# aai-institute/USFlows

Hardware: AMD Instinct MI355X
Metric: log_prob samples/sec (whole node), 32-layer 784-dim flow, batch 65536 (higher is better)
Workload: dtype f32 (GEMMs as bf16x3 split on the bf16 MFMA: 24 significant bits, fp32 accumulate); 1 GPU; BASELINE cfg2: USFlow in_dims=[784], 32 additive coupling blocks, ConditionalDenseNN[256, 256]+LeakyReLU(0.01), lu_transform=1, householder=0, affine_conjugation=False, Laplace(0,1) base; log_prob of 65536 rows per GPU (65536 over 1 GPU(s)) resident in HBM; conditioned synthetic parameters (seed 100, alpha 0.1); rows_per_gpu=65536, global_rows=65536, parallelism=dp1 (single GPU: no collective), fused_coupling=True, gemm_mode=bf16x3, merge_affine=auto -> False; probe (accepted, element-wise, L1) []

## Files before the change

### usflows_amd/csrc/usf_coupling_planes.hip

```cpp
#include <stdlib.h>

#include <type_traits>

#include "usf_common.h"

namespace usf {

typedef __bf16 cp_bf16x8 __attribute__((ext_vector_type(8)));
typedef _Float16 cp_f16x8 __attribute__((ext_vector_type(8)));
#define USF_CP_F16_GUARD 65000.0f
#ifndef USF_CP_ADDR32
#define USF_CP_ADDR32 1
#endif

__device__ __forceinline__ void cp_pin(unsigned& off) { asm("" : "+v"(off)); }
template <class V> __device__ __forceinline__ V cp_load(const void* uniform, unsigned off) {
  return *reinterpret_cast<const V*>(reinterpret_cast<const char*>(uniform) + off);
}
template <class V> __device__ __forceinline__ void cp_store(void* uniform, unsigned off, const V v) {
  *reinterpret_cast<V*>(reinterpret_cast<char*>(uniform) + off) = v;
}

__device__ __forceinline__ float max_with_product(float x, float sx) {
  float r;
  asm("v_max_f32 %0, %1, %2" : "=v"(r) : "v"(x), "v"(sx));
  return r;
}

template <int NPL> struct CPlanes;
template <> struct CPlanes<3> {
  typedef cp_bf16x8 vec;
  static __device__ __forceinline__ f32x4 mfma(vec a, vec b, f32x4 c) { return __builtin_amdgcn_mfma_f32_16x16x32_bf16(a, b, c, 0, 0, 0); }
  static __device__ __forceinline__ void split(const f32x4 x0, const f32x4 x1, vec (&o)[3]) {
#pragma unroll
    for (int j = 0; j < 8; ++j) {
      const float x = (j < 4) ? x0[j & 3] : x1[j & 3];
      const __bf16 h = (__bf16)x;
      const float r = x - (float)h;
      const __bf16 m = (__bf16)r;
      o[0][j] = h; o[1][j] = m; o[2][j] = (__bf16)(r - (float)m);
    }
  }
  static __device__ __forceinline__ void split1(const float x, const int j, vec (&o)[3]) {
    const __bf16 h = (__bf16)x;
    const float r = x - (float)h;
    const __bf16 m = (__bf16)r;
    o[0][j] = h; o[1][j] = m; o[2][j] = (__bf16)(r - (float)m);
  }
  static __device__ __forceinline__ void mm(f32x4& acc, const vec (&w)[3], const vec (&a)[3]) {
    acc = mfma(w[2], a[0], acc); acc = mfma(w[1], a[1], acc); acc = mfma(w[0], a[2], acc);
    acc = mfma(w[1], a[0], acc); acc = mfma(w[0], a[1], acc); acc = mfma(w[0], a[0], acc);
  }
};
template <> struct CPlanes<2> {
  typedef cp_f16x8 vec;
  static __device__ __forceinline__ f32x4 mfma(vec a, vec b, f32x4 c) { return __builtin_amdgcn_mfma_f32_16x16x32_f16(a, b, c, 0, 0, 0); }
  static __device__ __forceinline__ void split(const f32x4 x0, const f32x4 x1, vec (&o)[2]) {
#pragma unroll
    for (int j = 0; j < 8; ++j) {
      const float x = (j < 4) ? x0[j & 3] : x1[j & 3];
      const _Float16 h = (_Float16)x;
      o[0][j] = h; o[1][j] = (_Float16)(x - (float)h);
    }
  }
  static __device__ __forceinline__ void split1(const float x, const int j, vec (&o)[2]) {
    const _Float16 h = (_Float16)x;
    o[0][j] = h; o[1][j] = (_Float16)(x - (float)h);
  }
  static __device__ __forceinline__ void mm(f32x4& acc, const vec (&w)[2], const vec (&a)[2]) {
    acc = mfma(w[1], a[0], acc); acc = mfma(w[0], a[1], acc); acc = mfma(w[0], a[0], acc);
  }
};

struct CplPArgs {
  char* z; int z_nkb, npanels, M;
  int kb_p0, nk_p, kb_t0, nk_t;
  const char* Win; int64_t ld_in, pl_in; const float* b_in;
  const char* Whid[2]; int64_t ld_hid, pl_hid; const float* b_hid[2];
  const char* Wout; int64_t ld_out, pl_out; const float* b_out;
  float sign, slope; int act;
  int act_max;
  int32_t* range_flag;
  int descend;
  unsigned long long* dbg;
  char* hout[2]; const char* gate[2];
  const float* ctx; int ctx_stride; const float* w_ctx; const float* b_ctx;
  const char* side;
};

#ifdef USF_STAMP
#define CSTAMP(v) unsigned long long v = __builtin_amdgcn_s_memtime(); __builtin_amdgcn_sched_barrier(0)
#else
#define CSTAMP(v)
#endif

template <int NPL, int NH, int MODE = 0, bool CTX = false, bool SIDE = false>
__global__ __launch_bounds__(512, 2) void coupling_planes_kernel(const CplPArgs p) {
  static_assert(!SIDE || (MODE == 0 && !CTX), "the fp32 residual serves the plain inference launch");
  typedef CPlanes<NPL> PT;
  typedef typename PT::vec vec8;
  constexpr int T = 16;
  constexpr int HP = 16 * T;
  constexpr int KS = T / 2;
  constexpr int NT = 512;
  constexpr int SLOTS = NPL * 4 * HP;
  constexpr int NST = SLOTS / NT;
  constexpr int NPP = NST / NPL;
  constexpr int NC = HP / 8;
  constexpr int NPR = (NPL == 3) ? 6 : 3;
#ifndef USF_CP_AHEAD
#define USF_CP_AHEAD 3
#endif
  constexpr int AHEAD = USF_CP_AHEAD;
  __shared__ __attribute__((aligned(16))) float lds[2][SLOTS * 4];

  const int tid = threadIdx.x;
  const int lane = tid & 63;
  constexpr bool A32 = USF_CP_ADDR32 != 0;
  const int wave = A32 ? __builtin_amdgcn_readfirstlane(tid >> 6) : (tid >> 6);
  const int lj = lane & 15, lg = lane >> 4;
  unsigned loff = (unsigned)lane * 16u;
  unsigned goff = (unsigned)lg * 16u;
  const int panel = (p.descend ? (int)(gridDim.x - 1 - blockIdx.x) : (int)blockIdx.x) * 8 + wave;
  const int panc = min(panel, p.npanels - 1);
  const bool live = panel < p.npanels;
  const bool live_z = CTX ? (live && 16 * panel + lj < p.M) : live;
  const f32x4 zero4 = {0.f, 0.f, 0.f, 0.f};
  constexpr unsigned CHB = NPL * 1024u;
  const size_t zbase = ((size_t)panc * p.z_nkb) * CHB + (size_t)lane * 16;
  char* const zrow = p.z + ((size_t)panc * p.z_nkb) * CHB;
  auto k_off = [&](int64_t ld) { return 2u * ((unsigned)(tid >> 2) * (unsigned)ld + 8u * (unsigned)(tid & 3)); };
  auto n_off = [&](int64_t ld) { return 2u * ((unsigned)(tid / NC) * (unsigned)ld + 8u * (unsigned)(tid % NC)); };

  int kdst[NPP];
  unsigned krow[NPP];
#pragma unroll
  for (int i = 0; i < NPP; ++i) {
    const int idx = tid + NT * i;
    const int r = idx >> 2, c = idx & 3;
    kdst[i] = 4 * (c * HP + (r ^ (2 * c)));
    krow[i] = (unsigned)r;
  }
  auto issue_k = [&](const char* W, int64_t ld, int64_t pl, int k0, unsigned& off, f32x4 (&st)[NST]) {
    if constexpr (A32) cp_pin(off);
#pragma unroll
    for (int q = 0; q < NPL; ++q)
#pragma unroll
      for (int i = 0; i < NPP; ++i) {
        if constexpr (A32)
          st[q * NPP + i] = cp_load<f32x4>(W + 2 * (q * pl + (int64_t)((NT / 4) * i) * ld + k0), off);
        else
          st[q * NPP + i] = *reinterpret_cast<const f32x4*>(W + 2 * (q * pl + (int64_t)krow[i] * ld + k0 + 8 * ((tid + NT * i) & 3)));
      }
  };
  auto store_k = [&](int buf, const f32x4 (&st)[NST]) {
#pragma unroll
    for (int q = 0; q < NPL; ++q)
#pragma unroll
      for (int i = 0; i < NPP; ++i) *reinterpret_cast<f32x4*>(&lds[buf][q * 16 * HP + kdst[i]]) = st[q * NPP + i];
  };
  auto n_rc = [&](int i, int& r, int& c) { const int idx = tid + NT * i; r = idx / NC; c = idx % NC; };
  auto issue_n = [&](const char* W, int64_t ld, int64_t pl, int n0, unsigned& off, f32x4 (&st)[NST]) {
    if constexpr (A32) cp_pin(off);
#pragma unroll
    for (int q = 0; q < NPL; ++q)
#pragma unroll
      for (int i = 0; i < NPP; ++i) {
        if constexpr (A32) {
          st[q * NPP + i] = cp_load<f32x4>(W + 2 * (q * pl + (int64_t)(n0 + (NT / NC) * i) * ld), off);
        } else {
          int r, c; n_rc(i, r, c);
          st[q * NPP + i] = *reinterpret_cast<const f32x4*>(W + 2 * (q * pl + (int64_t)(n0 + r) * ld + 8 * c));
        }
      }
  };
  auto store_n = [&](int buf, const f32x4 (&st)[NST]) {
#pragma unroll
    for (int q = 0; q < NPL; ++q)
#pragma unroll
      for (int i = 0; i < NPP; ++i) {
        int r, c; n_rc(i, r, c);
        *reinterpret_cast<f32x4*>(&lds[buf][4 * ((q * NC + c) * 32 + (r ^ (2 * (c & 7))))]) = st[q * NPP + i];
      }
  };

  auto bias4 = [&](const float* b, int t) {
    if constexpr (A32) { if (t == 0) cp_pin(goff); return cp_load<f32x4>(b + t * 16, goff); }
    else return *reinterpret_cast<const f32x4*>(b + t * 16 + 4 * lg);
  };
  f32x4 X1[T], X2[T];
#pragma unroll
  for (int t = 0; t < T; ++t) X1[t] = bias4(p.b_in, t);
  if (CTX) {
    const int crow = min(16 * panc + lj, p.M - 1);
    const float c = p.ctx[(size_t)crow * p.ctx_stride];
#pragma unroll
    for (int t = 0; t < T; ++t) {
      const f32x4 wc = *reinterpret_cast<const f32x4*>(p.w_ctx + t * 16 + 4 * lg);
      const f32x4 bc = *reinterpret_cast<const f32x4*>(p.b_ctx + t * 16 + 4 * lg);
#pragma unroll
      for (int e = 0; e < 4; ++e) X1[t][e] = __builtin_fmaf(c, wc[e], X1[t][e] + bc[e]);
    }
  }

  auto load_z = [&](int kb, vec8 (&dst)[NPL]) {
    if constexpr (A32) cp_pin(loff);
#pragma unroll
    for (int q = 0; q < NPL; ++q) {
      if constexpr (A32) dst[q] = cp_load<vec8>(zrow + ((size_t)(p.kb_p0 + kb) * CHB + q * 1024), loff);
      else dst[q] = *reinterpret_cast<const vec8*>(p.z + zbase + (size_t)(p.kb_p0 + kb) * CHB + q * 1024);
    }
  };

  auto mfma_slab = [&](int buf, f32x4 (&X)[T], const vec8 (&b)[NPL]) {
    const float* wl = &lds[buf][4 * (lg * HP + (lj ^ (2 * lg)))];
#pragma unroll
    for (int ht = 0; ht < T; ++ht) {
      vec8 w[NPL];
#pragma unroll
      for (int q = 0; q < NPL; ++q) w[q] = *reinterpret_cast<const vec8*>(wl + 4 * ((q * 4) * HP + ht * 16));
#ifndef USF_CP_NOPRIO
      if (ht & 1) __builtin_amdgcn_s_setprio(0); else __builtin_amdgcn_s_setprio(1);
#endif
      PT::mm(X[ht], w, b);
    }
  };
#define CP_PIN_SLAB(NLD, VPT)                                                                     \
  do {                                                                                            \
    __builtin_amdgcn_sched_group_barrier(0x100, NPL * AHEAD, 0);                                  \
    _Pragma("unroll") for (int ht_ = 0; ht_ < T; ++ht_) {                                         \
      __builtin_amdgcn_sched_group_barrier(0x008, NPR, 0);                                        \
      if (ht_ + AHEAD < T) __builtin_amdgcn_sched_group_barrier(0x100, NPL, 0);                   \
      if (ht_ < (NLD)) __builtin_amdgcn_sched_group_barrier(0x020, 1, 0);                         \
      if (ht_ >= 3 && (VPT) > 0) __builtin_amdgcn_sched_group_barrier(0x002, (VPT), 0);           \
    }                                                                                             \
  } while (0)

  bool bad = false;
  auto guard = [&](const f32x4 v) {
    if (NPL == 2) {
#pragma unroll
      for (int j = 0; j < 4; ++j) bad = bad || !(fabsf(v[j]) < USF_CP_F16_GUARD);
    }
  };

  CSTAMP(c0);
  int g = 0;
  f32x4 st[NST];
  vec8 zp[NPL], zn[NPL];
  unsigned koff_in = k_off(p.ld_in), koff_hid = k_off(p.ld_hid), noff = n_off(p.ld_out);
  issue_k(p.Win, p.ld_in, p.pl_in, 0, koff_in, st);
  load_z(0, zp);
  store_k(0, st);
  __syncthreads();

  for (int s = 0; s + 1 < p.nk_p; ++s, ++g) {
    const int buf = g & 1;
    issue_k(p.Win, p.ld_in, p.pl_in, (s + 1) * 32, koff_in, st);
    load_z(s + 1, zn);
    mfma_slab(buf, X1, zp);
    CP_PIN_SLAB(NST + NPL, 0);
    __builtin_amdgcn_sched_barrier(0);
    store_k(buf ^ 1, st);
#pragma unroll
    for (int q = 0; q < NPL; ++q) zp[q] = zn[q];
    __syncthreads();
  }
  {
    const int buf = g & 1;
    if (NH >= 2) issue_k(p.Whid[0], p.ld_hid, p.pl_hid, 0, koff_hid, st); else issue_n(p.Wout, p.ld_out, p.pl_out, 0, noff, st);
    mfma_slab(buf, X1, zp);
    CP_PIN_SLAB(NST, 0);
    __builtin_amdgcn_sched_barrier(0);
    if (NH >= 2) store_k(buf ^ 1, st); else store_n(buf ^ 1, st);
    __syncthreads();
    ++g;
  }
  const size_t hbase = (size_t)panc * 8 * CHB + (size_t)lane * 16;
  const size_t hrow = (size_t)panc * 8 * CHB;
  auto activate = [&](f32x4 (&X)[T], int l) {
    if (MODE == 2) {
      if constexpr (A32) cp_pin(loff);
#pragma unroll
      for (int ks = 0; ks < KS; ++ks) {
        const vec8 hv = A32 ? cp_load<vec8>(p.gate[l] + (hrow + (size_t)ks * CHB), loff)
                            : *reinterpret_cast<const vec8*>(p.gate[l] + hbase + (size_t)ks * CHB);
#pragma unroll
        for (int t = 0; t < 4; ++t) {
          X[2 * ks][t] = gate_apply(X[2 * ks][t], (float)hv[t], p.slope);
          X[2 * ks + 1][t] = gate_apply(X[2 * ks + 1][t], (float)hv[4 + t], p.slope);
        }
      }
      return;
    }
    if (p.act_max) {
#pragma unroll
      for (int ht = 0; ht < T; ++ht) {
#pragma unroll
        for (int t = 0; t < 4; ++t) X[ht][t] = max_with_product(X[ht][t], X[ht][t] * p.slope);
        guard(X[ht]);
      }
      return;
    }
#pragma unroll
    for (int ht = 0; ht < T; ++ht) {
#pragma unroll
      for (int t = 0; t < 4; ++t) X[ht][t] = act_apply(X[ht][t], p.act, p.slope);
      guard(X[ht]);
    }
  };
  auto save_hidden = [&](int l, int ks, const vec8 (&x)[NPL]) {
    if (MODE != 0 && live) {
      if constexpr (A32) cp_pin(loff);
#pragma unroll
      for (int q = 0; q < NPL; ++q) {
        if constexpr (A32) cp_store<vec8>(p.hout[l] + (hrow + (size_t)ks * CHB + q * 1024), loff, x[q]);
        else *reinterpret_cast<vec8*>(p.hout[l] + hbase + (size_t)ks * CHB + q * 1024) = x[q];
      }
    }
  };
  activate(X1, 0);
  CSTAMP(c1);

  auto hidden_layer = [&](f32x4 (&Xin)[T], f32x4 (&Xout)[T], int l) {
    vec8 xc[NPL], xn[NPL];
    PT::split(Xin[0], Xin[1], xc);
#pragma unroll
    for (int ks = 0; ks < KS; ++ks) {
      save_hidden(l, ks, xc);
      const int buf = g & 1;
      const bool last = (ks + 1 == KS);
      const bool next_is_hidden = (l + 2 < NH);
      if (!last) issue_k(p.Whid[l], p.ld_hid, p.pl_hid, (ks + 1) * 32, koff_hid, st);
      else if (next_is_hidden) issue_k(p.Whid[l + 1], p.ld_hid, p.pl_hid, 0, koff_hid, st);
      else issue_n(p.Wout, p.ld_out, p.pl_out, 0, noff, st);
      mfma_slab(buf, Xout, xc);
      if (!last) PT::split(Xin[2 * ks + 2], Xin[2 * ks + 3], xn);
      CP_PIN_SLAB(NST, (NPL == 3) ? 5 : 3);
      __builtin_amdgcn_sched_barrier(0);
      if (!last || next_is_hidden) store_k(buf ^ 1, st); else store_n(buf ^ 1, st);
      if (!last) {
#pragma unroll
        for (int q = 0; q < NPL; ++q) xc[q] = xn[q];
      }
      __syncthreads();
      ++g;
    }
    activate(Xout, l + 1);
  };
  if (NH >= 2) {
#pragma unroll
    for (int t = 0; t < T; ++t) X2[t] = bias4(p.b_hid[0], t);
    hidden_layer(X1, X2, 0);
  }
  if (NH >= 3) {
#pragma unroll
    for (int t = 0; t < T; ++t) X1[t] = bias4(p.b_hid[1], t);
    hidden_layer(X2, X1, 1);
  }

  CSTAMP(c2);
  auto output_layer = [&](f32x4 (&X)[T]) {
    vec8 xp[KS][NPL];
#pragma unroll
    for (int ks = 0; ks < KS; ++ks) { PT::split(X[2 * ks], X[2 * ks + 1], xp[ks]); save_hidden(NH - 1, ks, xp[ks]); }
    typename std::conditional<SIDE, f32x4, vec8>::type res[SIDE ? 2 : NPL];
    f32x4 bo[2];
    unsigned soff = (unsigned)lane * 32u;
    const char* const srow = SIDE ? p.side + ((size_t)panc * p.nk_t) * 2048u : nullptr;
    auto issue_res = [&](int nt) {
      if constexpr (A32) { cp_pin(loff); cp_pin(goff); }
      if constexpr (SIDE) {
        if constexpr (A32) cp_pin(soff);
#pragma unroll
        for (int u = 0; u < 2; ++u) res[u] = cp_load<f32x4>(srow + ((size_t)nt * 2048u + 16 * u), soff);
      } else {
#pragma unroll
        for (int q = 0; q < NPL; ++q) {
          if constexpr (A32) res[q] = cp_load<vec8>(zrow + ((size_t)(p.kb_t0 + nt) * CHB + q * 1024), loff);
          else res[q] = *reinterpret_cast<const vec8*>(p.z + zbase + (size_t)(p.kb_t0 + nt) * CHB + q * 1024);
        }
      }
#pragma unroll
      for (int u = 0; u < 2; ++u) {
        if constexpr (A32) bo[u] = cp_load<f32x4>(p.b_out + nt * 32 + 16 * u, goff);
        else bo[u] = *reinterpret_cast<const f32x4*>(p.b_out + nt * 32 + 16 * u + 4 * lg);
      }
    };
    auto epilogue = [&](int nt, const auto& ac, const auto& rs) {
      f32x4 v[2];
#pragma unroll
      for (int u = 0; u < 2; ++u) {
#pragma unroll
        for (int e = 0; e < 4; ++e) {
          float r;
          if constexpr (SIDE) {
            r = rs[u][e];
          } else {
            r = (float)rs[0][4 * u + e] + (float)rs[1][4 * u + e];
            if (NPL == 3) r = r + (float)rs[NPL - 1][4 * u + e];
          }
          v[u][e] = __builtin_fmaf(p.sign, ac[u][e], r);
        }
        guard(v[u]);
      }
      vec8 o[NPL];
      PT::split(v[0], v[1], o);
      if (live_z) {
        if constexpr (A32) cp_pin(loff);
#pragma unroll
        for (int q = 0; q < NPL; ++q) {
          if constexpr (A32) cp_store<vec8>(zrow + ((size_t)(p.kb_t0 + nt) * CHB + q * 1024), loff, o[q]);
          else *reinterpret_cast<vec8*>(p.z + zbase + (size_t)(p.kb_t0 + nt) * CHB + q * 1024) = o[q];
        }
      }
    };
    issue_res(0);
    auto block = [&](int nt) {
      const int buf = g & 1;
      issue_n(p.Wout, p.ld_out, p.pl_out, min(nt + 1, p.nk_t - 1) * 32, noff, st);
      f32x4 acc[2] = {bo[0], bo[1]};
#pragma unroll
      for (int ks = 0; ks < KS; ++ks) {
        const int x = 2 * ((4 * ks + lg) & 7);
#pragma unroll
        for (int u = 0; u < 2; ++u) {
          const float* wf = &lds[buf][4 * ((4 * ks + lg) * 32 + u * 16 + (lj ^ x))];
          vec8 w[NPL];
#pragma unroll
          for (int q = 0; q < NPL; ++q) w[q] = *reinterpret_cast<const vec8*>(wf + 4 * (q * NC * 32));
          PT::mm(acc[u], w, xp[ks]);
        }
      }
      __builtin_amdgcn_sched_group_barrier(0x100, NPL * AHEAD, 0);
#pragma unroll
      for (int i = 0; i < 2 * KS; ++i) {
        __builtin_amdgcn_sched_group_barrier(0x008, NPR, 0);
        if (i + AHEAD < 2 * KS) __builtin_amdgcn_sched_group_barrier(0x100, NPL, 0);
        if (i < NST + (SIDE ? 2 : NPL) + 2) __builtin_amdgcn_sched_group_barrier(0x020, 1, 0);
      }
      __builtin_amdgcn_sched_barrier(0);
      store_n(buf ^ 1, st);
      epilogue(nt, acc, res);
      issue_res(min(nt + 1, p.nk_t - 1));
      __syncthreads();
      ++g;
    };
    for (int nt = 0; nt < p.nk_t; ++nt) block(nt);
  };
  if (NH == 2) output_layer(X2); else output_layer(X1);
#ifdef USF_STAMP
  CSTAMP(c3);
  if (p.dbg && lane == 0) {
    unsigned long long* o = p.dbg + (size_t)((blockIdx.x % 2048) * 8 + wave) * 4;
    o[0] = c1 - c0; o[1] = c2 - c1; o[2] = c3 - c2; o[3] = 1;
  }
#endif
  if (NPL == 2 && p.range_flag && bad && live && (16 * panel + lj) < p.M) atomicOr(p.range_flag, 1);
#undef CP_PIN_SLAB
}



#ifdef USF_STAMP
unsigned long long* g_cdbg = nullptr;
#endif

static int coupling_planes_launch(const usf_coupling_planes_desc* d, const float* ctx, int64_t ctx_stride, const float* w_ctx,
                                  const float* b_ctx, const void* side, int64_t side_nkb, hipStream_t stream) {
  if (!d) { set_error("usf_coupling_planes: null descriptor"); return -1; }
  if (ctx) {
    if (d->act == USF_ACT_GATE) { set_error("usf_coupling_planes_ctx: USF_ACT_GATE takes no context (the context enters no data gradient)"); return -2; }
    if (ctx_stride != 0 && ctx_stride != 1) { set_error("usf_coupling_planes_ctx: ctx_stride must be 0 or 1 (got %lld)", (long long)ctx_stride); return -2; }
    if (!w_ctx || !b_ctx || !aligned16(w_ctx) || !aligned16(b_ctx)) {
      set_error("usf_coupling_planes_ctx: w_ctx / b_ctx must be [256] fp32 vectors, 16-byte aligned");
      return -2;
    }
  }
  if (d->M < 0 || d->M > 0x7fffffff || d->z_nkb <= 0 || d->n_hidden < 1 || d->n_hidden > 3 || d->nk_p <= 0 || d->nk_t <= 0 ||
      d->kb_p0 < 0 || d->kb_t0 < 0 || d->kb_p0 + d->nk_p > d->z_nkb || d->kb_t0 + d->nk_t > d->z_nkb) {
    set_error("usf_coupling_planes: bad sizes / block ranges");
    return -2;
  }
  if (d->M == 0) return 0;
  if (d->format != USF_PLANES_BF16X3 && d->format != USF_PLANES_F16X2) { set_error("usf_coupling_planes: unknown format %d", d->format); return -2; }
  if (!d->z || !d->W_in || !d->W_out || !d->b_in || !d->b_out) { set_error("usf_coupling_planes: null pointer"); return -1; }
  for (int i = 0; i + 1 < d->n_hidden; ++i)
    if (!d->W_hid[i] || !d->b_hid[i]) { set_error("usf_coupling_planes: hidden layer %d missing", i); return -1; }
  if (d->hidden_padded != 256) { set_error("usf_coupling_planes: weights must be padded to a hidden width of 256 (got %d)", d->hidden_padded); return -2; }
  if (d->ldw_in < 32 * d->nk_p || (d->n_hidden > 1 && d->ldw_hid < 256) || d->ldw_out < 256 || (d->ldw_in & 7) || (d->ldw_hid & 7) ||
      (d->ldw_out & 7) || !aligned16(d->z) || !aligned16(d->W_in) || !aligned16(d->W_out) || !aligned16(d->b_in) || !aligned16(d->b_out)) {
    set_error("usf_coupling_planes: weight-image contract violated (ldw_in >= 32 nk_p, ldw_hid / ldw_out >= 256, multiples of 8, 16-byte aligned)");
    return -2;
  }
  const int64_t npl = d->format == USF_PLANES_F16X2 ? 2 : 3;
  const int64_t npanels = (d->M + 15) / 16;
  if (2 * npl * d->w_in_plane >= (1LL << 40)) { set_error("usf_coupling_planes: operand too large"); return -3; }
  {
    const int64_t lim = 1LL << 32, chb = npl * 1024;
    const bool z_big = d->z_nkb >= lim / chb || npanels * d->z_nkb * chb >= lim;
    const bool h_big = (d->hidden_out[0] || d->hidden_out[1]) && npanels * 8 * chb >= lim;
    auto w_big = [&](int64_t ld, int64_t plane, int64_t rows) {
      return ld < 0 || plane < 0 || ld >= lim / (2 * rows) || plane >= lim / (2 * npl);
    };
    if (z_big || h_big || w_big(d->ldw_in, d->w_in_plane, 256) || (d->n_hidden > 1 && w_big(d->ldw_hid, d->w_hid_plane, 256)) ||
        w_big(d->ldw_out, d->w_out_plane, 32 * d->nk_t)) {
      set_error("usf_coupling_planes: a buffer of 4 GiB or more (z: %lld panels x %lld blocks x %lld bytes; weights: ld %lld / %lld / %lld)",
                (long long)npanels, (long long)d->z_nkb, (long long)chb, (long long)d->ldw_in, (long long)d->ldw_hid, (long long)d->ldw_out);
      return -3;
    }
  }
  if (side) {
    if (ctx || d->hidden_out[0] || d->hidden_out[1] || d->act == USF_ACT_GATE) {
      set_error("usf_coupling_planes_side: the fp32 residual serves the inference launch without a context (no hidden_out, no USF_ACT_GATE)");
      return -2;
    }
    if (!aligned16(side)) { set_error("usf_coupling_planes_side: side must be 16-byte aligned"); return -2; }
    if (side_nkb != d->nk_t) {
      set_error("usf_coupling_planes_side: the side buffer holds %lld blocks per panel, the layer transforms %lld", (long long)side_nkb, (long long)d->nk_t);
      return -2;
    }
    if (npanels * d->nk_t * 2048 >= (1LL << 32)) { set_error("usf_coupling_planes_side: side buffer of 4 GiB or more"); return -3; }
  }
  CplPArgs a;
  a.side = reinterpret_cast<const char*>(side);
  a.z = reinterpret_cast<char*>(d->z); a.z_nkb = (int)d->z_nkb; a.npanels = (int)npanels; a.M = (int)d->M;
  a.kb_p0 = (int)d->kb_p0; a.nk_p = (int)d->nk_p; a.kb_t0 = (int)d->kb_t0; a.nk_t = (int)d->nk_t;
  a.Win = reinterpret_cast<const char*>(d->W_in); a.ld_in = d->ldw_in; a.pl_in = d->w_in_plane; a.b_in = d->b_in;
  for (int i = 0; i < 2; ++i) {
    const bool used = i + 1 < d->n_hidden;
    a.Whid[i] = reinterpret_cast<const char*>(used ? d->W_hid[i] : d->W_in);
    a.b_hid[i] = used ? d->b_hid[i] : d->b_in;
  }
  a.ld_hid = d->ldw_hid; a.pl_hid = d->w_hid_plane;
  a.Wout = reinterpret_cast<const char*>(d->W_out); a.ld_out = d->ldw_out; a.pl_out = d->w_out_plane; a.b_out = d->b_out;
  a.sign = d->sign; a.slope = d->slope; a.act = d->act; a.range_flag = d->range_flag;
  a.act_max = (d->act == USF_ACT_LEAKY_RELU && d->slope >= 0.0f && d->slope <= 1.0f && !__builtin_signbit(d->slope) &&
               tuning("coupling_act_max", 1) != 0) ? 1 : 0;
  a.descend = (int)tuning("coupling_descend", 1);
  a.ctx = ctx; a.ctx_stride = (int)ctx_stride; a.w_ctx = w_ctx; a.b_ctx = b_ctx;
  a.dbg = nullptr;
#ifdef USF_STAMP
  a.dbg = g_cdbg;
#endif
  const dim3 grid((unsigned)((npanels + 7) / 8));
  const bool want_h = d->hidden_out[0] != nullptr || d->hidden_out[1] != nullptr;
  const bool gated = d->act == USF_ACT_GATE;
  if (d->act != USF_ACT_NONE && d->act != USF_ACT_LEAKY_RELU && !gated) { set_error("usf_coupling_planes: bad act %d", d->act); return -2; }
  for (int i = 0; i < 2; ++i) { a.hout[i] = nullptr; a.gate[i] = nullptr; }
  if (want_h || gated) {
    if (npl != 3 || d->n_hidden > 2) { set_error("usf_coupling_planes: hidden_out / USF_ACT_GATE need the bf16x3 format and n_hidden <= 2"); return -2; }
    if (gated && !want_h) { set_error("usf_coupling_planes: USF_ACT_GATE needs hidden_out (the gradients at the hidden pre-activations)"); return -2; }
    for (int i = 0; i < d->n_hidden; ++i) {
      if (!d->hidden_out[i] || !aligned16(d->hidden_out[i]) || (gated && (!d->gate[i] || !aligned16(d->gate[i])))) {
        set_error("usf_coupling_planes: hidden_out[l] (and gate[l] with USF_ACT_GATE) must be set for every hidden layer, 16-byte aligned");
        return -2;
      }
      a.hout[i] = reinterpret_cast<char*>(d->hidden_out[i]);
      a.gate[i] = reinterpret_cast<const char*>(gated ? d->gate[i] : nullptr);
    }
    const dim3 block(512);
#define USF_CPT(NH_, MODE_) hipLaunchKernelGGL((coupling_planes_kernel<3, NH_, MODE_>), grid, block, 0, stream, a)
#define USF_CPTC(NH_) hipLaunchKernelGGL((coupling_planes_kernel<3, NH_, 1, true>), grid, block, 0, stream, a)
    if (gated) { if (d->n_hidden == 1) USF_CPT(1, 2); else USF_CPT(2, 2); }
    else if (ctx) { if (d->n_hidden == 1) USF_CPTC(1); else USF_CPTC(2); }
    else { if (d->n_hidden == 1) USF_CPT(1, 1); else USF_CPT(2, 1); }
#undef USF_CPTC
#undef USF_CPT
    return check_launch("usf_coupling_planes");
  }
  const dim3 block(512);
#define USF_CPL(NPL_, NH_) hipLaunchKernelGGL((coupling_planes_kernel<NPL_, NH_>), grid, block, 0, stream, a)
#define USF_CPLC(NPL_, NH_) hipLaunchKernelGGL((coupling_planes_kernel<NPL_, NH_, 0, true>), grid, block, 0, stream, a)
#define USF_CPLS(NPL_, NH_) hipLaunchKernelGGL((coupling_planes_kernel<NPL_, NH_, 0, false, true>), grid, block, 0, stream, a)
  if (side) {
    if (npl == 2) {
      switch (d->n_hidden) { case 1: USF_CPLS(2, 1); break; case 2: USF_CPLS(2, 2); break; default: USF_CPLS(2, 3); break; }
    } else {
      switch (d->n_hidden) { case 1: USF_CPLS(3, 1); break; case 2: USF_CPLS(3, 2); break; default: USF_CPLS(3, 3); break; }
    }
  } else if (ctx) {
    if (npl == 2) {
      switch (d->n_hidden) { case 1: USF_CPLC(2, 1); break; case 2: USF_CPLC(2, 2); break; default: USF_CPLC(2, 3); break; }
    } else {
      switch (d->n_hidden) { case 1: USF_CPLC(3, 1); break; case 2: USF_CPLC(3, 2); break; default: USF_CPLC(3, 3); break; }
    }
  } else if (npl == 2) {
    switch (d->n_hidden) { case 1: USF_CPL(2, 1); break; case 2: USF_CPL(2, 2); break; default: USF_CPL(2, 3); break; }
  } else {
    switch (d->n_hidden) { case 1: USF_CPL(3, 1); break; case 2: USF_CPL(3, 2); break; default: USF_CPL(3, 3); break; }
  }
#undef USF_CPLS
#undef USF_CPLC
#undef USF_CPL
  return check_launch("usf_coupling_planes");
}

int coupling_planes_ctx(const usf_coupling_planes_desc* d, const float* ctx, int64_t ctx_stride, const float* w_ctx,
                        const float* b_ctx, hipStream_t stream) {
  return coupling_planes_launch(d, ctx, ctx_stride, w_ctx, b_ctx, nullptr, 0, stream);
}

int coupling_planes_side(const usf_coupling_planes_desc* d, const void* side, int64_t side_nkb, hipStream_t stream) {
  return coupling_planes_launch(d, nullptr, 0, nullptr, nullptr, side, side_nkb, stream);
}

int coupling_planes(const usf_coupling_planes_desc* d, hipStream_t stream) { return coupling_planes_ctx(d, nullptr, 0, nullptr, nullptr, stream); }

}
```

Baseline: 3.507 million samples/s.

## Pipeline coupling-kernel weight staging through a three-slot LDS ring with mid-stage barrier

Replaces the double-buffered LDS weight staging with a three-slot ring. Global weight loads are issued two stages ahead and LDS stores are interleaved into the first half of each MFMA stage, with the block barrier moved to mid-stage. Fragments for the next stage are prefetched across the stage boundary, and the default lookahead drops to 2 for the three-plane path. The intent is to hide global-load and barrier latency behind MFMA work. In exchange it uses 1.5x the LDS, adds register pressure from the carried fragments, and could reduce occupancy under launch_bounds(512,2). It also drops the live guard on hidden saves.

```diff
diff --git a/usflows_amd/csrc/usf_coupling_planes.hip b/usflows_amd/csrc/usf_coupling_planes.hip
--- a/usflows_amd/csrc/usf_coupling_planes.hip
+++ b/usflows_amd/csrc/usf_coupling_planes.hip
@@ -14,6 +14,7 @@
 #endif
 
 __device__ __forceinline__ void cp_pin(unsigned& off) { asm("" : "+v"(off)); }
+__device__ __forceinline__ void cp_fence() { asm volatile("" ::: "memory"); }
 template <class V> __device__ __forceinline__ V cp_load(const void* uniform, unsigned off) {
   return *reinterpret_cast<const V*>(reinterpret_cast<const char*>(uniform) + off);
 }
@@ -108,11 +109,12 @@
   constexpr int NPP = NST / NPL;
   constexpr int NC = HP / 8;
   constexpr int NPR = (NPL == 3) ? 6 : 3;
-#ifndef USF_CP_AHEAD
-#define USF_CP_AHEAD 3
-#endif
+#ifdef USF_CP_AHEAD
   constexpr int AHEAD = USF_CP_AHEAD;
-  __shared__ __attribute__((aligned(16))) float lds[2][SLOTS * 4];
+#else
+  constexpr int AHEAD = (NPL == 3) ? 2 : 3;
+#endif
+  __shared__ __attribute__((aligned(16))) float lds[3][SLOTS * 4];
 
   const int tid = threadIdx.x;
   const int lane = tid & 63;
@@ -125,64 +127,57 @@
   const int panc = min(panel, p.npanels - 1);
   const bool live = panel < p.npanels;
   const bool live_z = CTX ? (live && 16 * panel + lj < p.M) : live;
-  const f32x4 zero4 = {0.f, 0.f, 0.f, 0.f};
   constexpr unsigned CHB = NPL * 1024u;
   const size_t zbase = ((size_t)panc * p.z_nkb) * CHB + (size_t)lane * 16;
   char* const zrow = p.z + ((size_t)panc * p.z_nkb) * CHB;
   auto k_off = [&](int64_t ld) { return 2u * ((unsigned)(tid >> 2) * (unsigned)ld + 8u * (unsigned)(tid & 3)); };
   auto n_off = [&](int64_t ld) { return 2u * ((unsigned)(tid / NC) * (unsigned)ld + 8u * (unsigned)(tid % NC)); };
 
-  int kdst[NPP];
-  unsigned krow[NPP];
-#pragma unroll
-  for (int i = 0; i < NPP; ++i) {
-    const int idx = tid + NT * i;
-    const int r = idx >> 2, c = idx & 3;
-    kdst[i] = 4 * (c * HP + (r ^ (2 * c)));
-    krow[i] = (unsigned)r;
-  }
-  auto issue_k = [&](const char* W, int64_t ld, int64_t pl, int k0, unsigned& off, f32x4 (&st)[NST]) {
+  constexpr int RH = 8 * (NH - 1);
+  const int kdst = 4 * ((tid & 3) * HP + ((tid >> 2) ^ (2 * (tid & 3))));
+  const int ndst = 4 * ((tid % NC) * 32 + ((tid / NC) ^ (2 * ((tid % NC) & 7))));
+  constexpr int KDI = 4 * (NT / 4), NDI = 4 * (NT / NC);
+  static_assert(NT / 4 >= 8 && NT / NC >= 16 && (NT / NC) * NPP <= 32, "the row swizzle stays inside a thread's first row's low bits");
+  static_assert(NC * 32 * 4 == 16 * HP, "k-slab and n-tile images share the plane stride");
+  unsigned koff_in = k_off(p.ld_in), koff_hid = k_off(p.ld_hid), noff = n_off(p.ld_out);
+  auto issue_from = [&](const char* base, int64_t rstep, int64_t pstep, unsigned& off, f32x4 (&st)[NST]) {
     if constexpr (A32) cp_pin(off);
 #pragma unroll
     for (int q = 0; q < NPL; ++q)
 #pragma unroll
-      for (int i = 0; i < NPP; ++i) {
-        if constexpr (A32)
-          st[q * NPP + i] = cp_load<f32x4>(W + 2 * (q * pl + (int64_t)((NT / 4) * i) * ld + k0), off);
-        else
-          st[q * NPP + i] = *reinterpret_cast<const f32x4*>(W + 2 * (q * pl + (int64_t)krow[i] * ld + k0 + 8 * ((tid + NT * i) & 3)));
-      }
-  };
-  auto store_k = [&](int buf, const f32x4 (&st)[NST]) {
-#pragma unroll
-    for (int q = 0; q < NPL; ++q)
-#pragma unroll
-      for (int i = 0; i < NPP; ++i) *reinterpret_cast<f32x4*>(&lds[buf][q * 16 * HP + kdst[i]]) = st[q * NPP + i];
-  };
-  auto n_rc = [&](int i, int& r, int& c) { const int idx = tid + NT * i; r = idx / NC; c = idx % NC; };
-  auto issue_n = [&](const char* W, int64_t ld, int64_t pl, int n0, unsigned& off, f32x4 (&st)[NST]) {
-    if constexpr (A32) cp_pin(off);
-#pragma unroll
-    for (int q = 0; q < NPL; ++q)
-#pragma unroll
-      for (int i = 0; i < NPP; ++i) {
-        if constexpr (A32) {
-          st[q * NPP + i] = cp_load<f32x4>(W + 2 * (q * pl + (int64_t)(n0 + (NT / NC) * i) * ld), off);
-        } else {
-          int r, c; n_rc(i, r, c);
-          st[q * NPP + i] = *reinterpret_cast<const f32x4*>(W + 2 * (q * pl + (int64_t)(n0 + r) * ld + 8 * c));
-        }
-      }
-  };
-  auto store_n = [&](int buf, const f32x4 (&st)[NST]) {
-#pragma unroll
-    for (int q = 0; q < NPL; ++q)
-#pragma unroll
-      for (int i = 0; i < NPP; ++i) {
-        int r, c; n_rc(i, r, c);
-        *reinterpret_cast<f32x4*>(&lds[buf][4 * ((q * NC + c) * 32 + (r ^ (2 * (c & 7))))]) = st[q * NPP + i];
-      }
-  };
+      for (int i = 0; i < NPP; ++i) st[q * NPP + i] = cp_load<f32x4>(base + q * pstep + i * rstep, off);
+  };
+  auto issue_stage = [&](int r, f32x4 (&st)[NST]) {
+    if (r < 0) {
+      issue_from(p.Win + 2 * (int64_t)(p.nk_p + r) * 32, 2 * (NT / 4) * p.ld_in, 2 * p.pl_in, koff_in, st);
+    } else if (r < RH) {
+      issue_from(p.Whid[r >> 3] + 2 * (r & 7) * 32, 2 * (NT / 4) * p.ld_hid, 2 * p.pl_hid, koff_hid, st);
+    } else {
+      const int nt = min(r - RH, p.nk_t - 1);
+      issue_from(p.Wout + 2 * (int64_t)(nt * 32) * p.ld_out, 2 * (NT / NC) * p.ld_out, 2 * p.pl_out, noff, st);
+    }
+  };
+  auto store_one = [&](bool n, int s, int j, const f32x4 (&st)[NST]) {
+    const int q = j / NPP, i = j % NPP;
+    *reinterpret_cast<f32x4*>(&lds[s][q * 16 * HP + (n ? ndst + NDI * i : kdst + KDI * i)]) = st[j];
+  };
+  auto store_stage = [&](bool n, int s, const f32x4 (&st)[NST]) {
+#pragma unroll
+    for (int j = 0; j < NST; ++j) store_one(n, s, j, st);
+  };
+  auto frag = [&](bool n, int s, int i, vec8 (&w)[NPL]) {
+    const float* wl;
+    if (n) {
+      const int ks = i >> 1, u = i & 1;
+      const int x = 2 * ((4 * ks + lg) & 7);
+      wl = &lds[s][4 * ((4 * ks + lg) * 32 + u * 16 + (lj ^ x))];
+    } else {
+      wl = &lds[s][4 * (lg * HP + (lj ^ (2 * lg)) + i * 16)];
+    }
+#pragma unroll
+    for (int q = 0; q < NPL; ++q) w[q] = *reinterpret_cast<const vec8*>(wl + q * 16 * HP);
+  };
+  auto ring_next = [](int s) { return s == 2 ? 0 : s + 1; };
 
   auto bias4 = [&](const float* b, int t) {
     if constexpr (A32) { if (t == 0) cp_pin(goff); return cp_load<f32x4>(b + t * 16, goff); }
@@ -212,30 +207,6 @@
     }
   };
 
-  auto mfma_slab = [&](int buf, f32x4 (&X)[T], const vec8 (&b)[NPL]) {
-    const float* wl = &lds[buf][4 * (lg * HP + (lj ^ (2 * lg)))];
-#pragma unroll
-    for (int ht = 0; ht < T; ++ht) {
-      vec8 w[NPL];
-#pragma unroll
-      for (int q = 0; q < NPL; ++q) w[q] = *reinterpret_cast<const vec8*>(wl + 4 * ((q * 4) * HP + ht * 16));
-#ifndef USF_CP_NOPRIO
-      if (ht & 1) __builtin_amdgcn_s_setprio(0); else __builtin_amdgcn_s_setprio(1);
-#endif
-      PT::mm(X[ht], w, b);
-    }
-  };
-#define CP_PIN_SLAB(NLD, VPT)                                                                     \
-  do {                                                                                            \
-    __builtin_amdgcn_sched_group_barrier(0x100, NPL * AHEAD, 0);                                  \
-    _Pragma("unroll") for (int ht_ = 0; ht_ < T; ++ht_) {                                         \
-      __builtin_amdgcn_sched_group_barrier(0x008, NPR, 0);                                        \
-      if (ht_ + AHEAD < T) __builtin_amdgcn_sched_group_barrier(0x100, NPL, 0);                   \
-      if (ht_ < (NLD)) __builtin_amdgcn_sched_group_barrier(0x020, 1, 0);                         \
-      if (ht_ >= 3 && (VPT) > 0) __builtin_amdgcn_sched_group_barrier(0x002, (VPT), 0);           \
-    }                                                                                             \
-  } while (0)
-
   bool bad = false;
   auto guard = [&](const f32x4 v) {
     if (NPL == 2) {
@@ -244,37 +215,83 @@
     }
   };
 
+  static_assert(AHEAD >= 1 && AHEAD <= T / 2, "the first half of a stage reads its own slot only");
+  f32x4 st[NST];
+  vec8 wf[AHEAD][NPL];
+  int slot = 0;
+  constexpr int ST0 = (T / 2 - NST) / 2;
+#define CP_PIN_HALF(FIRST, NLD, VPT, V0)                                                          \
+  do {                                                                                            \
+    _Pragma("unroll") for (int i_ = 0; i_ < T / 2; ++i_) {                                        \
+      __builtin_amdgcn_sched_group_barrier(0x008, NPR, 0);                                        \
+      __builtin_amdgcn_sched_group_barrier(0x100, NPL, 0);                                        \
+      if ((FIRST) && i_ >= ST0 && i_ < ST0 + NST) __builtin_amdgcn_sched_group_barrier(0x200, 1, 0); \
+      if (i_ < (NLD)) __builtin_amdgcn_sched_group_barrier(0x020, 1, 0);                          \
+      if (i_ >= (V0) && (VPT) > 0) __builtin_amdgcn_sched_group_barrier(0x002, (VPT), 0);         \
+    }                                                                                             \
+  } while (0)
+  auto k_stage = [&](f32x4 (&X)[T], const vec8 (&b)[NPL], int r, bool next_n, auto nld_c, auto vpt_c, auto&& front, auto&& back) {
+    constexpr int NLDA = decltype(nld_c)::value, VPT = decltype(vpt_c)::value;
+    const int nslot = ring_next(slot);
+    vec8 w[T + AHEAD][NPL];
+#pragma unroll
+    for (int i = 0; i < AHEAD; ++i)
+#pragma unroll
+      for (int q = 0; q < NPL; ++q) w[i][q] = wf[i][q];
+    front();
+#pragma unroll
+    for (int ht = 0; ht < T / 2; ++ht) {
+      frag(false, slot, ht + AHEAD, w[ht + AHEAD]);
+#ifndef USF_CP_NOPRIO
+      if (ht & 1) __builtin_amdgcn_s_setprio(0); else __builtin_amdgcn_s_setprio(1);
+#endif
+      PT::mm(X[ht], w[ht], b);
+      if (ht >= ST0 && ht < ST0 + NST) store_one(next_n, nslot, ht - ST0, st);
+    }
+    CP_PIN_HALF(true, NLDA, VPT, 1);
+    __builtin_amdgcn_sched_barrier(0);
+    __syncthreads();
+    __builtin_amdgcn_sched_barrier(0);
+    back();
+    issue_stage(r + 2, st);
+#pragma unroll
+    for (int ht = T / 2; ht < T; ++ht) {
+      if (ht + AHEAD < T) frag(false, slot, ht + AHEAD, w[ht + AHEAD]); else frag(next_n, nslot, ht + AHEAD - T, w[ht + AHEAD]);
+#ifndef USF_CP_NOPRIO
+      if (ht & 1) __builtin_amdgcn_s_setprio(0); else __builtin_amdgcn_s_setprio(1);
+#endif
+      PT::mm(X[ht], w[ht], b);
+    }
+    CP_PIN_HALF(false, NST, VPT, 0);
+    __builtin_amdgcn_sched_barrier(0);
+    cp_fence();
+#pragma unroll
+    for (int i = 0; i < AHEAD; ++i)
+#pragma unroll
+      for (int q = 0; q < NPL; ++q) wf[i][q] = w[T + i][q];
+    slot = nslot;
+  };
+  const std::integral_constant<int, 0> no_c{};
+
   CSTAMP(c0);
-  int g = 0;
-  f32x4 st[NST];
   vec8 zp[NPL], zn[NPL];
-  unsigned koff_in = k_off(p.ld_in), koff_hid = k_off(p.ld_hid), noff = n_off(p.ld_out);
-  issue_k(p.Win, p.ld_in, p.pl_in, 0, koff_in, st);
+  issue_stage(-p.nk_p, st);
   load_z(0, zp);
-  store_k(0, st);
+  store_stage(false, 0, st);
+  issue_stage(1 - p.nk_p, st);
   __syncthreads();
-
-  for (int s = 0; s + 1 < p.nk_p; ++s, ++g) {
-    const int buf = g & 1;
-    issue_k(p.Win, p.ld_in, p.pl_in, (s + 1) * 32, koff_in, st);
-    load_z(s + 1, zn);
-    mfma_slab(buf, X1, zp);
-    CP_PIN_SLAB(NST + NPL, 0);
-    __builtin_amdgcn_sched_barrier(0);
-    store_k(buf ^ 1, st);
-#pragma unroll
-    for (int q = 0; q < NPL; ++q) zp[q] = zn[q];
-    __syncthreads();
-  }
+#pragma unroll
+  for (int i = 0; i < AHEAD; ++i) frag(false, 0, i, wf[i]);
+
   {
-    const int buf = g & 1;
-    if (NH >= 2) issue_k(p.Whid[0], p.ld_hid, p.pl_hid, 0, koff_hid, st); else issue_n(p.Wout, p.ld_out, p.pl_out, 0, noff, st);
-    mfma_slab(buf, X1, zp);
-    CP_PIN_SLAB(NST, 0);
-    __builtin_amdgcn_sched_barrier(0);
-    if (NH >= 2) store_k(buf ^ 1, st); else store_n(buf ^ 1, st);
-    __syncthreads();
-    ++g;
+    const int n1 = (NH == 1) ? p.nk_p - 1 : p.nk_p;
+    for (int s = 0; s < n1; ++s) {
+      k_stage(X1, zp, s - p.nk_p, false, std::integral_constant<int, NPL>{}, no_c,
+              [&] { load_z(min(s + 1, p.nk_p - 1), zn); }, [] {});
+#pragma unroll
+      for (int q = 0; q < NPL; ++q) zp[q] = zn[q];
+    }
+    if (NH == 1) k_stage(X1, zp, -1, true, no_c, no_c, [] {}, [] {});
   }
   const size_t hbase = (size_t)panc * 8 * CHB + (size_t)lane * 16;
   const size_t hrow = (size_t)panc * 8 * CHB;
@@ -310,7 +327,7 @@
     }
   };
   auto save_hidden = [&](int l, int ks, const vec8 (&x)[NPL]) {
-    if (MODE != 0 && live) {
+    if (MODE != 0) {
       if constexpr (A32) cp_pin(loff);
 #pragma unroll
       for (int q = 0; q < NPL; ++q) {
@@ -320,6 +337,7 @@
     }
   };
   activate(X1, 0);
+  if (MODE == 2) __builtin_amdgcn_sched_barrier(0);
   CSTAMP(c1);
 
   auto hidden_layer = [&](f32x4 (&Xin)[T], f32x4 (&Xout)[T], int l) {
@@ -327,24 +345,26 @@
     PT::split(Xin[0], Xin[1], xc);
 #pragma unroll
     for (int ks = 0; ks < KS; ++ks) {
-      save_hidden(l, ks, xc);
-      const int buf = g & 1;
       const bool last = (ks + 1 == KS);
-      const bool next_is_hidden = (l + 2 < NH);
-      if (!last) issue_k(p.Whid[l], p.ld_hid, p.pl_hid, (ks + 1) * 32, koff_hid, st);
-      else if (next_is_hidden) issue_k(p.Whid[l + 1], p.ld_hid, p.pl_hid, 0, koff_hid, st);
-      else issue_n(p.Wout, p.ld_out, p.pl_out, 0, noff, st);
-      mfma_slab(buf, Xout, xc);
-      if (!last) PT::split(Xin[2 * ks + 2], Xin[2 * ks + 3], xn);
-      CP_PIN_SLAB(NST, (NPL == 3) ? 5 : 3);
-      __builtin_amdgcn_sched_barrier(0);
-      if (!last || next_is_hidden) store_k(buf ^ 1, st); else store_n(buf ^ 1, st);
+      const int r = 8 * l + ks;
+      k_stage(Xout, xc, r, r + 1 >= RH, no_c, std::integral_constant<int, (NPL == 3) ? 5 : 3>{},
+              [&] {
+                save_hidden(l, ks, xc);
+                if (!last) {
+#pragma unroll
+                  for (int j = 0; j < 4; ++j) PT::split1(Xin[2 * ks + 2][j], j, xn);
+                }
+              },
+              [&] {
+                if (!last) {
+#pragma unroll
+                  for (int j = 0; j < 4; ++j) PT::split1(Xin[2 * ks + 3][j], 4 + j, xn);
+                }
+              });
       if (!last) {
 #pragma unroll
         for (int q = 0; q < NPL; ++q) xc[q] = xn[q];
       }
-      __syncthreads();
-      ++g;
     }
     activate(Xout, l + 1);
   };
@@ -362,14 +382,12 @@
   CSTAMP(c2);
   auto output_layer = [&](f32x4 (&X)[T]) {
     vec8 xp[KS][NPL];
-#pragma unroll
-    for (int ks = 0; ks < KS; ++ks) { PT::split(X[2 * ks], X[2 * ks + 1], xp[ks]); save_hidden(NH - 1, ks, xp[ks]); }
     typename std::conditional<SIDE, f32x4, vec8>::type res[SIDE ? 2 : NPL];
     f32x4 bo[2];
     unsigned soff = (unsigned)lane * 32u;
     const char* const srow = SIDE ? p.side + ((size_t)panc * p.nk_t) * 2048u : nullptr;
     auto issue_res = [&](int nt) {
-      if constexpr (A32) { cp_pin(loff); cp_pin(goff); }
+      if constexpr (A32) cp_pin(loff);
       if constexpr (SIDE) {
         if constexpr (A32) cp_pin(soff);
 #pragma unroll
@@ -381,6 +399,9 @@
           else res[q] = *reinterpret_cast<const vec8*>(p.z + zbase + (size_t)(p.kb_t0 + nt) * CHB + q * 1024);
         }
       }
+    };
+    auto issue_bias = [&](int nt) {
+      if constexpr (A32) cp_pin(goff);
 #pragma unroll
       for (int u = 0; u < 2; ++u) {
         if constexpr (A32) bo[u] = cp_load<f32x4>(p.b_out + nt * 32 + 16 * u, goff);
@@ -415,40 +436,53 @@
         }
       }
     };
+    issue_bias(0);
+#pragma unroll
+    for (int ks = 0; ks < KS; ++ks) { PT::split(X[2 * ks], X[2 * ks + 1], xp[ks]); save_hidden(NH - 1, ks, xp[ks]); }
+    asm volatile("" : "+v"(bo[0]), "+v"(bo[1]));
     issue_res(0);
     auto block = [&](int nt) {
-      const int buf = g & 1;
-      issue_n(p.Wout, p.ld_out, p.pl_out, min(nt + 1, p.nk_t - 1) * 32, noff, st);
+      const int nslot = ring_next(slot);
       f32x4 acc[2] = {bo[0], bo[1]};
-#pragma unroll
-      for (int ks = 0; ks < KS; ++ks) {
-        const int x = 2 * ((4 * ks + lg) & 7);
-#pragma unroll
-        for (int u = 0; u < 2; ++u) {
-          const float* wf = &lds[buf][4 * ((4 * ks + lg) * 32 + u * 16 + (lj ^ x))];
-          vec8 w[NPL];
-#pragma unroll
-          for (int q = 0; q < NPL; ++q) w[q] = *reinterpret_cast<const vec8*>(wf + 4 * (q * NC * 32));
-          PT::mm(acc[u], w, xp[ks]);
-        }
-      }
-      __builtin_amdgcn_sched_group_barrier(0x100, NPL * AHEAD, 0);
-#pragma unroll
-      for (int i = 0; i < 2 * KS; ++i) {
-        __builtin_amdgcn_sched_group_barrier(0x008, NPR, 0);
-        if (i + AHEAD < 2 * KS) __builtin_amdgcn_sched_group_barrier(0x100, NPL, 0);
-        if (i < NST + (SIDE ? 2 : NPL) + 2) __builtin_amdgcn_sched_group_barrier(0x020, 1, 0);
-      }
+      vec8 w[2 * KS + AHEAD][NPL];
+#pragma unroll
+      for (int i = 0; i < AHEAD; ++i)
+#pragma unroll
+        for (int q = 0; q < NPL; ++q) w[i][q] = wf[i][q];
+#pragma unroll
+      for (int i = 0; i < KS; ++i) {
+        frag(true, slot, i + AHEAD, w[i + AHEAD]);
+        PT::mm(acc[i & 1], w[i], xp[i >> 1]);
+        if (i >= ST0 && i < ST0 + NST) store_one(true, nslot, i - ST0, st);
+      }
+      CP_PIN_HALF(true, 0, 0, 0);
       __builtin_amdgcn_sched_barrier(0);
-      store_n(buf ^ 1, st);
+      __syncthreads();
+      __builtin_amdgcn_sched_barrier(0);
+      issue_stage(RH + nt + 2, st);
+      issue_bias(min(nt + 1, p.nk_t - 1));
+#pragma unroll
+      for (int i = KS; i < 2 * KS; ++i) {
+        if (i + AHEAD < 2 * KS) frag(true, slot, i + AHEAD, w[i + AHEAD]); else frag(true, nslot, i + AHEAD - 2 * KS, w[i + AHEAD]);
+        PT::mm(acc[i & 1], w[i], xp[i >> 1]);
+      }
+      CP_PIN_HALF(false, NST + 2, 0, 0);
+      __builtin_amdgcn_sched_barrier(0);
+      cp_fence();
+      asm volatile("" : "+v"(bo[0]), "+v"(bo[1]));
       epilogue(nt, acc, res);
       issue_res(min(nt + 1, p.nk_t - 1));
-      __syncthreads();
-      ++g;
+      cp_fence();
+#pragma unroll
+      for (int i = 0; i < AHEAD; ++i)
+#pragma unroll
+        for (int q = 0; q < NPL; ++q) wf[i][q] = w[2 * KS + i][q];
+      slot = nslot;
     };
     for (int nt = 0; nt < p.nk_t; ++nt) block(nt);
   };
   if (NH == 2) output_layer(X2); else output_layer(X1);
+#undef CP_PIN_HALF
 #ifdef USF_STAMP
   CSTAMP(c3);
   if (p.dbg && lane == 0) {
@@ -457,7 +491,6 @@
   }
 #endif
   if (NPL == 2 && p.range_flag && bad && live && (16 * panel + lj) < p.M) atomicOr(p.range_flag, 1);
-#undef CP_PIN_SLAB
 }
 
 
```

Result: no change. 3.542 million samples/s, median of 6 (+1.0%).
